# unslothai/unsloth

Hardware: AMD Instinct MI355X
Metric: train tokens/sec, Llama-3-8B QLoRA (NF4) r=16 seq2048 bf16 (higher is better)
Workload: dtype bf16; 1 GPU; Llama-3-8B QLoRA NF4 r=16 (q,k,v,o,gate,up,down) seq2048 bf16, fwd+bwd+AdamW; model=Llama-3-8B (synthetic weights), global_batch=4, seq_len=2048, parallelism=dp1, layers=32, lora_rank=16, gradient_checkpointing=unsloth, gc_schedule_chosen=all (every layer keeps everything), nf4_decoded_weight_mirrors=off (every NF4 weight is decoded at every use INSIDE the timed step), trainable_params=41943040, attention=csrc/attention.hip (causal GQA flash, fwd+bwd), optimizer=FlatAdamW fp32 on LoRA params

## Files before the change

unsloth_amd/csrc/lora_side.hip:

```cpp
#include "common.h"

typedef __attribute__((ext_vector_type(2))) __bf16 bf16x2_t;
typedef __attribute__((ext_vector_type(2))) _Float16 f16x2_t;

#define UAMD_TN_MAX_PROBLEMS 8

namespace {

constexpr int TN_COLS = 128;
constexpr int TN_R = 16;

struct TnArgs {
    int n_probs;
    int M;
    int S;
    int rows_per_wave;
    int total_slabs;
    int slab_start[UAMD_TN_MAX_PROBLEMS + 1];
    int64_t ws_off[UAMD_TN_MAX_PROBLEMS];
    float* ws;
    uamd_lora_tn_problem p[UAMD_TN_MAX_PROBLEMS];
};

typedef __attribute__((ext_vector_type(8))) __bf16 bf16x8_t;
// ... 31 lines not shown
#endif
constexpr int TN_NST = UAMD_TN_STAGES;
static_assert(TN_NST >= 2 && TN_NST <= 4, "ring of 2..4 stages (4 x 4 x 10 KiB = the 160 KiB of a CU)");
constexpr int TN_WAVE_LDS = TN_NST * TN_STAGE;

__device__ __forceinline__ void tn_dma(const void* gptr, unsigned lds_dst) {
    unsigned keep;
    asm volatile(
        "s_mov_b32 %0, m0\n\t"
        "s_mov_b32 m0, %2\n\t"
        "s_nop 0\n\t"
        "global_load_lds_dwordx4 %1, off\n\t"
        "s_mov_b32 m0, %0"
        : "=&s"(keep)
        : "v"(gptr), "s"(lds_dst)
        : "memory");
}

template <typename T>
__global__ void __launch_bounds__(256) lora_tn_kernel(TnArgs a) {
    extern __shared__ __attribute__((aligned(16))) unsigned char smem[];
    typedef typename Mfma16<T>::frag frag_t;
    const int tid = threadIdx.x, lane = tid & 63;
    const int wave = __builtin_amdgcn_readfirstlane(tid >> 6);
    const int64_t unit = (int64_t)blockIdx.x * 4 + wave;
    if (unit >= (int64_t)a.total_slabs * a.S) return;
    const int slab_lin = (int)(unit % a.total_slabs);
    const int sblk = (int)(unit / a.total_slabs);
    int pi = 0;
#pragma unroll
    for (int i = 1; i < UAMD_TN_MAX_PROBLEMS; ++i)
        if (i < a.n_probs && slab_lin >= a.slab_start[i]) pi = i;
    const uamd_lora_tn_problem& pr = a.p[pi];
    const int slab = slab_lin - a.slab_start[pi];
    const int n_slabs = a.slab_start[pi + 1] - a.slab_start[pi];
    const int M = a.M, N = pr.N, R = pr.R;
    const T* Z = (const T*)pr.Z;
    const float* P = pr.P;
    unsigned char* my = smem + wave * TN_WAVE_LDS;
    const unsigned my_lds = (unsigned)(uintptr_t)(lds_u8*)my;

    const int zr4 = lane >> 4;
    int zcol[8];
#pragma unroll
    for (int i = 0; i < 8; ++i) {
        const int row = 4 * i + zr4;
        const int f = (row & 3) | (((row >> 3) & 1) << 2);
        const int u16 = ((((lane & 15) >> 1) ^ f) << 1) | (lane & 1);
        int col = slab * TN_COLS + u16 * 8;
        if (col + 8 > N) col = N - 8;
        zcol[i] = col;
    }
    const int prow = lane >> 2;
    const int pc = (lane & 3) * 4 + 4 <= ((R + 3) & ~3) ? (lane & 3) * 4 : 0;
    auto issue = [&](int m0, int stage) {
        const unsigned d = my_lds + stage * TN_STAGE;
#pragma unroll
        for (int i = 0; i < 8; ++i) {
            int row = m0 + 4 * i + zr4;
            row = row < M ? row : M - 1;
            tn_dma(Z + (int64_t)row * pr.ldz + zcol[i], d + i * 1024);
        }
#pragma unroll
        for (int i = 0; i < 2; ++i) {
            int row = m0 + 16 * i + prow;
            row = row < M ? row : M - 1;
            tn_dma(P + (int64_t)row * pr.ldp + pc, d + TN_ZT + i * 1024);
        }
    };

    const int l15 = lane & 15, g4 = lane >> 4;
    const int sg2 = l15 >> 2;
    const int f_rd = sg2 | ((g4 & 1) << 2);
    const int z_lane = (8 * g4 + sg2) * 256 + f_rd * 32 + (l15 & 3) * 8;
    const int p_lane = TN_ZT + (8 * g4) * 64 + l15 * 4;

    f32x4_t acc[8];
#pragma unroll
    for (int j = 0; j < 8; ++j) acc[j] = f32x4_t{0.f, 0.f, 0.f, 0.f};

    const int m_base = sblk * a.rows_per_wave;
    const int m_end = min(m_base + a.rows_per_wave, M);
    const int nch = (m_end - m_base + 31) / 32;
#pragma unroll
    for (int i = 0; i < TN_NST - 1; ++i)
        if (i < nch) issue(m_base + 32 * i, i);
    for (int ch = 0; ch < nch; ++ch) {
        const int m0 = m_base + ch * 32;
        const int stage = ch % TN_NST;
        if (ch + TN_NST - 1 < nch) {
            issue(m0 + 32 * (TN_NST - 1), (ch + TN_NST - 1) % TN_NST);
            if (TN_NST == 2) asm volatile("s_waitcnt vmcnt(10)" ::: "memory");
            else if (TN_NST == 3) asm volatile("s_waitcnt vmcnt(20)" ::: "memory");
            else asm volatile("s_waitcnt vmcnt(30)" ::: "memory");
        } else {
            const int younger = nch - 1 - ch;
            if (younger >= 2) asm volatile("s_waitcnt vmcnt(20)" ::: "memory");
            else if (younger == 1) asm volatile("s_waitcnt vmcnt(10)" ::: "memory");
            else asm volatile("s_waitcnt vmcnt(0)" ::: "memory");
        }
        const unsigned char* sz = my + stage * TN_STAGE;
        union { T e[8]; frag_t f; } pa;
#pragma unroll
        for (int e = 0; e < 8; ++e) {
            float x = *reinterpret_cast<const float*>(sz + p_lane + e * 64);
            if (m0 + 8 * g4 + e >= M || l15 >= R) x = 0.f;
            pa.e[e] = from_f32<T>(x);
        }
#pragma unroll
        for (int jt = 0; jt < 8; ++jt) {
            union { s16x4_t h[2]; frag_t f; } zb;
            const int a0 = z_lane ^ (jt * 32);
            zb.h[0] = __builtin_amdgcn_ds_read_tr16_b64_v4i16((lds_s16x4*)(sz + a0));
            zb.h[1] = __builtin_amdgcn_ds_read_tr16_b64_v4i16((lds_s16x4*)(sz + a0 + 4 * 256));
            acc[jt] = Mfma16<T>::run(pa.f, zb.f, acc[jt]);
        }
    }

    const int64_t npad = (int64_t)n_slabs * TN_COLS;
    float* part = a.ws + a.ws_off[pi] + (int64_t)sblk * TN_R * npad + slab * TN_COLS + l15;
#pragma unroll
    for (int jt = 0; jt < 8; ++jt)
#pragma unroll
        for (int r = 0; r < 4; ++r) part[(int64_t)(4 * g4 + r) * npad + jt * 16] = acc[jt][r];
}

__global__ void __launch_bounds__(256) lora_tn_reduce_kernel(TnArgs a) {
    const int pi = blockIdx.y;
    const uamd_lora_tn_problem& pr = a.p[pi];
    const int n_slabs = a.slab_start[pi + 1] - a.slab_start[pi];
    const int64_t npad = (int64_t)n_slabs * TN_COLS;
    const int64_t idx = (int64_t)blockIdx.x * 256 + threadIdx.x;
    const int N = pr.N, R = pr.R;
    if (idx >= (int64_t)R * N) return;
    const int r = (int)(idx / N), n = (int)(idx - (int64_t)r * N);
    const float* part = a.ws + a.ws_off[pi] + (int64_t)r * npad + n;
    float v = 0.f;
    const int64_t sstride = (int64_t)TN_R * npad;
    int s = 0;
    for (; s + 8 <= a.S; s += 8) {
        float t[8];
#pragma unroll
        for (int u = 0; u < 8; ++u) t[u] = part[(int64_t)(s + u) * sstride];
#pragma unroll
        for (int u = 0; u < 8; ++u) v += t[u];
    }
    for (; s < a.S; ++s) v += part[(int64_t)s * sstride];
    v *= pr.scale;
    float* o = (pr.out_nr & 1) ? pr.out + (int64_t)n * pr.ldo + r : pr.out + (int64_t)r * pr.ldo + n;
    *o = (pr.out_nr & 2) ? *o + v : v;
}

constexpr int XA_KS = 64;
constexpr int XA_XT = 32 * XA_KS * 2;
template <int NT> struct XaCfg {
    static constexpr int WT = NT * 16 * XA_KS * 2;
    static constexpr int STAGE = XA_XT + WT;
    static constexpr int WAVE = 2 * STAGE;
    static constexpr int RED = 4 * 32 * NT * 16 * 4;
    static constexpr int LDS = 4 * WAVE > RED ? 4 * WAVE : RED;
};

template <typename T, int NT>
__global__ void __launch_bounds__(256) lora_xa2_kernel(const T* __restrict__ X, int64_t ldx,
                                                       const T* __restrict__ W, int64_t ldw,
                                                       float* __restrict__ out, int64_t ld_out,
                                                       T* __restrict__ out_k, int64_t ld_k, int k_cols,
                                                       int M, int K, int R, int out_cols) {
    extern __shared__ __attribute__((aligned(16))) unsigned char smem[];
    typedef typename Mfma16<T>::frag frag_t;
    typedef XaCfg<NT> C;
    const int tid = threadIdx.x, lane = tid & 63;
    const int wave = __builtin_amdgcn_readfirstlane(tid >> 6);
    const int l15 = lane & 15, g4 = lane >> 4;
    const int m0 = blockIdx.x * 32;
    unsigned char* my = smem + wave * C::WAVE;
    const unsigned my_lds = (unsigned)(uintptr_t)(lds_u8*)my;

    const int nsteps_all = (K + XA_KS - 1) / XA_KS;
    const int s_beg = (nsteps_all * wave) / 4, s_end = (nsteps_all * (wave + 1)) / 4;

    const int drow = lane >> 3;
    int xoff[4], woff[2 * NT];
    int xslot[4];
#pragma unroll
    for (int i = 0; i < 4; ++i) {
        const int row = 8 * i + drow;
        xslot[i] = (lane & 7) ^ ((row >> 1) & 7);
        int gm = m0 + row;
        gm = gm < M ? gm : M - 1;
        xoff[i] = gm;
    }
    int wslot[2 * NT];
#pragma unroll
    for (int i = 0; i < 2 * NT; ++i) {
        const int row = 8 * i + drow;
        wslot[i] = (lane & 7) ^ ((row >> 1) & 7);
        woff[i] = row < R ? row : R - 1;
    }
    auto issue = [&](int step, int stage) {
        const unsigned d = my_lds + stage * C::STAGE;
        const int k0 = step * XA_KS;
#pragma unroll
        for (int i = 0; i < 4; ++i) {
            int k = k0 + xslot[i] * 8;
            k = k + 8 <= K ? k : K - 8;
            tn_dma(X + (int64_t)xoff[i] * ldx + k, d + i * 1024);
        }
#pragma unroll
        for (int i = 0; i < 2 * NT; ++i) {
            int k = k0 + wslot[i] * 8;
            k = k + 8 <= K ? k : K - 8;
            tn_dma(W + (int64_t)woff[i] * ldw + k, d + XA_XT + i * 1024);
        }
    };

    f32x4_t acc[2][NT];
#pragma unroll
    for (int i = 0; i < 2; ++i)
#pragma unroll
        for (int j = 0; j < NT; ++j) acc[i][j] = f32x4_t{0.f, 0.f, 0.f, 0.f};

    const int sw = (l15 >> 1) & 7;
    const int f_lane = l15 * 128;
    constexpr int NDMA = 4 + 2 * NT;
    const int nst = s_end - s_beg;
    const int rot = nst > 0 ? (int)(blockIdx.x % nst) : 0;
    auto step_of = [&](int i) { const int j = i + rot; return s_beg + (j >= nst ? j - nst : j); };
    if (nst > 0) issue(step_of(0), 0);
    for (int it = 0; it < nst; ++it) {
        const int st = step_of(it);
        const int stage = it & 1;
        if (it + 1 < nst) {
            issue(step_of(it + 1), stage ^ 1);
            if (NDMA == 6) asm volatile("s_waitcnt vmcnt(6)" ::: "memory");
            else if (NDMA == 8) asm volatile("s_waitcnt vmcnt(8)" ::: "memory");
            else if (NDMA == 10) asm volatile("s_waitcnt vmcnt(10)" ::: "memory");
            else asm volatile("s_waitcnt vmcnt(12)" ::: "memory");
        } else {
            asm volatile("s_waitcnt vmcnt(0)" ::: "memory");
        }
        const unsigned char* sx = my + stage * C::STAGE;
        const unsigned char* swt = sx + XA_XT;
        const bool tail = st * XA_KS + XA_KS > K;
#pragma unroll
        for (int ks = 0; ks < 2; ++ks) {
            const int slot = ((4 * ks + g4) ^ sw) * 16;
            union FU { uint4 r; frag_t f; };
            FU xa[2], wb[NT];
#pragma unroll
            for (int i = 0; i < 2; ++i) xa[i].r = *reinterpret_cast<const uint4*>(sx + i * 2048 + f_lane + slot);
#pragma unroll
            for (int j = 0; j < NT; ++j) wb[j].r = *reinterpret_cast<const uint4*>(swt + j * 2048 + f_lane + slot);
            if (tail) {
                if (st * XA_KS + ks * 32 + g4 * 8 + 8 > K) {
#pragma unroll
                    for (int i = 0; i < 2; ++i) xa[i].r = make_uint4(0, 0, 0, 0);
                }
            }
#pragma unroll
            for (int i = 0; i < 2; ++i)
#pragma unroll
                for (int j = 0; j < NT; ++j) acc[i][j] = Mfma16<T>::run(xa[i].f, wb[j].f, acc[i][j]);
        }
    }

    __syncthreads();
    float* red = reinterpret_cast<float*>(smem);
#pragma unroll
    for (int i = 0; i < 2; ++i)
#pragma unroll
        for (int j = 0; j < NT; ++j)
#pragma unroll
            for (int r = 0; r < 4; ++r)
                red[(wave * 32 + i * 16 + 4 * g4 + r) * (NT * 16) + j * 16 + l15] = acc[i][j][r];
    __syncthreads();
    if (out != nullptr) {
        for (int idx = tid; idx < 32 * out_cols; idx += 256) {
            const int mm = idx / out_cols, c = idx - mm * out_cols;
            if (m0 + mm < M) {
                float v = 0.f;
                if (c < R) {
                    const float* q = red + mm * (NT * 16) + c;
                    v = ((q[0] + q[32 * NT * 16]) + q[2 * 32 * NT * 16]) + q[3 * 32 * NT * 16];
                }
                out[(int64_t)(m0 + mm) * ld_out + c] = v;
            }
        }
    }
    if (out_k != nullptr) {
        const int vec_per_row = k_cols >> 3;
        for (int idx = tid; idx < 32 * vec_per_row; idx += 256) {
            const int mm = idx / vec_per_row, c0 = (idx - mm * vec_per_row) * 8;
            if (m0 + mm < M) {
                Vec16<T> v;
#pragma unroll
                for (int j = 0; j < 8; ++j) {
                    const int c = c0 + j;
                    float x = 0.f;
                    if (c < R) {
                        const float* q = red + mm * (NT * 16) + c;
                        x = ((q[0] + q[32 * NT * 16]) + q[2 * 32 * NT * 16]) + q[3 * 32 * NT * 16];
                    }
                    v.e[j] = from_f32<T>(x);
                }
                st16(out_k + (int64_t)(m0 + mm) * ld_k + c0, v);
            }
        }
    }
}

template <typename T, int NT>
int launch_xa2(const void* X, int64_t ldx, const void* W, int64_t ldw, float* out, int64_t ld_out, void* out_k,
               int64_t ld_k, int k_cols, int M, int K, int R, int out_cols, hipStream_t st) {
    return uamd_launch_lds<&lora_xa2_kernel<T, NT>>(dim3((unsigned)((M + 31) / 32)), dim3(256), XaCfg<NT>::LDS, st, (const T*)X, ldx,
                                                    (const T*)W, ldw, out, ld_out, (T*)out_k, ld_k, k_cols, M, K, R, out_cols);
}

template <typename T>
int xa2_dispatch(const void* X, int64_t ldx, const void* W, int64_t ldw, float* out, int64_t ld_out, void* out_k,
                 int64_t ld_k, int k_cols, int M, int K, int R, int out_cols, hipStream_t st) {
    const int nt = (R + 15) / 16;
    if (nt <= 1) return launch_xa2<T, 1>(X, ldx, W, ldw, out, ld_out, out_k, ld_k, k_cols, M, K, R, out_cols, st);
    if (nt <= 2) return launch_xa2<T, 2>(X, ldx, W, ldw, out, ld_out, out_k, ld_k, k_cols, M, K, R, out_cols, st);
    if (nt <= 3) return launch_xa2<T, 3>(X, ldx, W, ldw, out, ld_out, out_k, ld_k, k_cols, M, K, R, out_cols, st);
    if (nt <= 4) return launch_xa2<T, 4>(X, ldx, W, ldw, out, ld_out, out_k, ld_k, k_cols, M, K, R, out_cols, st);
    return UAMD_ERR_ARG;
}

}

extern "C" int uamd_lora_tn(const uamd_lora_tn_problem* probs, int n_probs, int M, float* workspace,
                            int64_t workspace_floats, int dtype, void* stream) {
    if (!probs || n_probs < 1 || n_probs > UAMD_TN_MAX_PROBLEMS || M < 0 || !workspace) return UAMD_ERR_ARG;
    if (M == 0) return UAMD_OK;
    TnArgs a;
    a.n_probs = n_probs; a.M = M; a.ws = workspace;
    {
        int64_t slabs_all = 0;
        for (int i = 0; i < n_probs; ++i) slabs_all += (probs[i].N + TN_COLS - 1) / TN_COLS;
        int rpw = UAMD_TN_RPW_MAX;
        while (rpw > 128 && slabs_all * ((M + rpw - 1) / rpw) < UAMD_TN_MIN_WAVES) rpw >>= 1;
        a.rows_per_wave = rpw;
        a.S = (M + rpw - 1) / rpw;
    }
    int slabs = 0;
    int64_t off = 0;
    int max_rn_blocks = 1;
    for (int i = 0; i < UAMD_TN_MAX_PROBLEMS; ++i) {
        a.slab_start[i] = slabs;
        if (i < n_probs) {
            const uamd_lora_tn_problem& p = probs[i];
            if (!p.P || !p.Z || !p.out || p.N <= 0 || p.R <= 0 || p.R > TN_R) return UAMD_ERR_ARG;
            if ((p.N & 7) || p.N < 8 || (p.ldz & 7) || (p.ldp & 3) || !aligned16(p.Z) || !aligned16(p.P)) return UAMD_ERR_ALIGN;
            a.p[i] = p;
            a.ws_off[i] = off;
            const int ns = (p.N + TN_COLS - 1) / TN_COLS;
            slabs += ns;
            off += (int64_t)a.S * TN_R * ns * TN_COLS;
            const int64_t rn = ((int64_t)p.R * p.N + 255) / 256;
            if (rn > max_rn_blocks) max_rn_blocks = (int)rn;
        } else {
            a.p[i] = probs[0];
            a.ws_off[i] = 0;
        }
    }
    a.slab_start[UAMD_TN_MAX_PROBLEMS] = slabs;
    for (int i = n_probs; i < UAMD_TN_MAX_PROBLEMS; ++i) a.slab_start[i + 1] = slabs;
    a.total_slabs = slabs;
    if (off > workspace_floats) return UAMD_ERR_ARG;
    const int64_t blocks = ((int64_t)slabs * a.S + 3) / 4;
    if (blocks > 0x7fffffffLL) return UAMD_ERR_ARG;
    hipStream_t st = (hipStream_t)stream;
    UAMD_DISPATCH_HALF(dtype,
        if (int rc = uamd_launch_lds<&lora_tn_kernel<T>>(dim3((unsigned)blocks), dim3(256), 4 * TN_WAVE_LDS, st, a)) return rc)
    hipLaunchKernelGGL(lora_tn_reduce_kernel, dim3((unsigned)max_rn_blocks, (unsigned)n_probs), dim3(256), 0, st, a);
    return uamd_launch_status();
}

extern "C" int uamd_lora_xa2k(const void* X, int64_t ldx, const void* W, int64_t ldw, float* out, int64_t ld_out,
                              void* out_k, int64_t ld_k, int k_cols, int M, int K, int R, int out_cols, int dtype,
                              void* stream) {
    if (M < 0 || K < 8 || R <= 0 || R > 64) return UAMD_ERR_ARG;
    if (!out && !out_k) return UAMD_ERR_ARG;
    if (out && (out_cols < R || out_cols > 256)) return UAMD_ERR_ARG;
    if (out_k && (k_cols < R || k_cols > 256)) return UAMD_ERR_ARG;
    if (M == 0) return UAMD_OK;
    if ((K & 7) || (ldx & 7) || (ldw & 7) || !aligned16(X) || !aligned16(W)) return UAMD_ERR_ALIGN;
    if (out_k && ((k_cols & 7) || (ld_k & 7) || !aligned16(out_k))) return UAMD_ERR_ALIGN;
    UAMD_DISPATCH_HALF(dtype, return xa2_dispatch<T>(X, ldx, W, ldw, out, ld_out, out_k, ld_k, k_cols, M, K, R, out_cols, (hipStream_t)stream))
    return UAMD_ERR_DTYPE;
}

extern "C" int uamd_lora_xa2(const void* X, int64_t ldx, const void* W, int64_t ldw, float* out, int64_t ld_out,
                             int M, int K, int R, int out_cols, int dtype, void* stream) {
    if (!out) return UAMD_ERR_ARG;
    return uamd_lora_xa2k(X, ldx, W, ldw, out, ld_out, nullptr, 0, 0, M, K, R, out_cols, dtype, stream);
}

namespace {
template <typename T>
__global__ void __launch_bounds__(256) lora_prepare_kernel(const uamd_lora_prep_desc* __restrict__ d, int n_mats,
                                                          const int* __restrict__ tile_prefix) {
    __shared__ float tile[32][33];
    int lo = 0, hi = n_mats - 1;
    const int bid = blockIdx.x;
    while (lo < hi) {
        const int mid = (lo + hi + 1) >> 1;
        if (tile_prefix[mid] <= bid) lo = mid; else hi = mid - 1;
    }
    const uamd_lora_prep_desc m = d[lo];
    const int t = bid - tile_prefix[lo];
    const int tiles_c = (m.cols + 31) / 32;
    const int r0 = (t / tiles_c) * 32, c0 = (t % tiles_c) * 32;
    const int tx = threadIdx.x & 31, ty = threadIdx.x >> 5;
    const float* src = (const float*)m.src;
    T* rm = (T*)m.dst_rowmajor;
    T* tr = (T*)m.dst_transposed;
    T* pad = (T*)m.dst_pad;
    const bool pad_t = m.pad_transposed != 0;
#pragma unroll
    for (int i = 0; i < 4; ++i) {
        const int r = r0 + ty + 8 * i, c = c0 + tx;
        float v = 0.f;
        if (r < m.rows && c < m.cols) {
            v = src[(int64_t)r * m.cols + c];
            if (rm) rm[(int64_t)r * m.cols + c] = from_f32<T>(v);
            if (pad && !pad_t) pad[(int64_t)r * m.pad_ld + c] = from_f32<T>(m.pad_scale * v);
        }
        tile[ty + 8 * i][tx] = v;
    }
    __syncthreads();
    if (tr || (pad && pad_t)) {
#pragma unroll
        for (int i = 0; i < 4; ++i) {
            const int c = c0 + ty + 8 * i, r = r0 + tx;
            if (r < m.rows && c < m.cols) {
                const float v = tile[tx][ty + 8 * i];
                if (tr) tr[(int64_t)c * m.rows + r] = from_f32<T>(v);
                if (pad && pad_t) pad[(int64_t)c * m.pad_ld + r] = from_f32<T>(m.pad_scale * v);
            }
        }
    }
}
}

extern "C" int uamd_lora_prepare(const uamd_lora_prep_desc* descs_dev, const int* tile_prefix_dev, int n_mats,
                                 int total_tiles, int dtype, void* stream) {
    if (!descs_dev || !tile_prefix_dev || n_mats <= 0 || total_tiles < 0) return UAMD_ERR_ARG;
    if (total_tiles == 0) return UAMD_OK;
    hipStream_t st = (hipStream_t)stream;
    UAMD_DISPATCH_HALF(dtype, hipLaunchKernelGGL((lora_prepare_kernel<T>), dim3((unsigned)total_tiles), dim3(256), 0, st, descs_dev, n_mats,
                                                 tile_prefix_dev))
    return uamd_launch_status();
}
```

unsloth_amd/kernels/utils.py:

```python
import ctypes
import os

import torch

from .. import _lib
from .. import nf4 as _nf4
from .._lib import GemmGroup

MAX_FUSED_SIZE = 65536
next_power_of_2 = lambda n: 1 << (max(int(n), 1) - 1).bit_length()

FUSED_NF4 = True
FUSED_NF4_MAX_M = 512
GEMM256_MODE = "auto"
GEMM256_MIN_TILES = 160
LORA_XA_V2 = True
LORA_XA_MAX_RANKS = 192


def calculate_settings(n):
    BLOCK_SIZE = next_power_of_2(n)
    num_warps = 4
    if BLOCK_SIZE >= 32768:
        num_warps = 32
# ... 60 lines not shown


def get_lora_parameters_bias(proj):
    base_layer = getattr(proj, "base_layer", proj)
    W = base_layer.weight
    W_quant = _resolve_quant_state(base_layer, W)
    if getattr(proj, "disable_adapters", True) or proj.merged:
        return W, W_quant, None, None, None, base_layer.bias
    adapter = getattr(proj, "active_adapters", None)
    if adapter is None:
        adapter = getattr(proj, "active_adapter", ("default"))
    adapter = adapter[0]
    return (W, W_quant, proj.lora_A[adapter].weight, proj.lora_B[adapter].weight,
            proj.scaling[adapter], base_layer.bias)


@torch.inference_mode()
def fast_dequantize(W, quant_state=None, out=None, use_global_buffer=False):
    if quant_state is None:
        return W
    _refuse_fp8([(W,)])
    is_transposed = W.shape[0] == 1
    packed = W.t() if is_transposed else W
    out = _nf4.dequantize_nf4(packed, quant_state, out=out, use_global_buffer=use_global_buffer)
    return out.t() if is_transposed else out


def _group(B, C, N, ldb, absmax=None, xa=None, ld_xa=0, lb=None, R=0, scale=0.0, xk=None, bk=None, bias=None):
    return GemmGroup(
        B=B.data_ptr(), C=C.data_ptr(), absmax=absmax.data_ptr() if absmax is not None else None,
        lora_xa=xa.data_ptr() if xa is not None else None, lora_b=lb.data_ptr() if lb is not None else None,
        ldb=ldb, ldc=C.stride(0), ld_xa=ld_xa, ld_lb=lb.stride(0) if lb is not None else 0,
        N=N, R=R, lora_scale=float(scale), _pad=0,
        lora_xk=xk.data_ptr() if xk is not None else None, lora_bk=bk.data_ptr() if bk is not None else None,
        ld_xk=xk.stride(0) if xk is not None else 0, ld_bk=bk.stride(0) if bk is not None else 0,
        Rk=xk.shape[1] if xk is not None else 0, _pad2=0, bias=bias.data_ptr() if bias is not None else None)


def _use_gemm256(M, K, Ns):
    if GEMM256_MODE == "off" or K % 64:
        return False
    if GEMM256_MODE == "on":
        return True
    cols = sum((n + 255) // 256 for n in Ns)
    return ((M + 255) // 256) * cols >= GEMM256_MIN_TILES or ((M + 127) // 128) * cols >= GEMM256_MIN_TILES


GEMM_SPAN_LIMIT = 1 << 32


def _chunk_rows(row_bytes, align):
    rows = (GEMM_SPAN_LIMIT - 1) // max(row_bytes, 1) // align * align
    if rows < align:
        raise RuntimeError(f"unsloth_amd: a GEMM operand row of {row_bytes} bytes leaves no whole {align}-row chunk "
                           f"below the {GEMM_SPAN_LIMIT}-byte span limit")
    return rows


def _row_spans(M, row_bytes, align):
    if M * row_bytes < GEMM_SPAN_LIMIT:
        return [(0, M)]
    step = _chunk_rows(row_bytes, align)
    return [(r0, min(step, M - r0)) for r0 in range(0, M, step)]


def _launch_gemm(X2d, groups, nf4, accumulate=False, nn=False):
    M, K = X2d.shape
    prologue_lora = any(g.lora_xa and not g.lora_xk for g in groups)
    if nn:
        name = "uamd_gemm_nn_256"
    elif nf4:
        name = "uamd_gemm_nt_nf4"
    elif _use_gemm256(M, K, [g.N for g in groups]) and not prologue_lora:
        name = "uamd_gemm_nt_256"
    else:
        name = "uamd_gemm_nt"
    item = X2d.element_size()
    row_bytes = X2d.stride(0) * item
    for g in groups:
        if g.lora_xk:
            row_bytes = max(row_bytes, g.ld_xk * item)
        if g.lora_xa:
            row_bytes = max(row_bytes, g.ld_xa * 4)
    for r0, rows in _row_spans(M, row_bytes, 256):
        chunk = []
        for g in groups:
            c = GemmGroup.from_buffer_copy(g)
            if r0:
                c.C += r0 * c.ldc * item
                if c.lora_xk:
                    c.lora_xk += r0 * c.ld_xk * item
                if c.lora_xa:
                    c.lora_xa += r0 * c.ld_xa * 4
            chunk.append(c)
        arr = (GemmGroup * len(chunk))(*chunk)
        _lib.call(name, X2d, ctypes.c_void_p(X2d.data_ptr() + r0 * X2d.stride(0) * item), X2d.stride(0), rows, K, arr,
                  len(chunk), int(accumulate), _lib.dtype_code(X2d.dtype), _lib.stream_of(X2d))
    return name


def _aligned_rows(W):
    return W.stride(1) == 1 and W.stride(0) % 8 == 0 and W.data_ptr() % 16 == 0


def _aligned_copy(W, dtype=None):
    Wc = W.to(dtype if dtype is not None else W.dtype).contiguous()
    return Wc.clone() if Wc.data_ptr() % 16 else Wc


def _rows2d(X):
    X2d = X.reshape(-1, X.shape[-1])
    return X2d if _aligned_rows(X2d) else _aligned_copy(X2d)


def _out2d(C, M, N, dtype, name):
    if not isinstance(C, torch.Tensor) or not C.is_cuda or C.dtype != dtype:
        raise ValueError(f"{name}: expected a {dtype} tensor on the GPU, got {getattr(C, 'dtype', type(C))}")
    C2 = C
    if C.dim() != 2 and C.dim() >= 1 and C.shape[-1] == N and C.numel() == M * N:
        try:
            C2 = C.view(M, N)
        except RuntimeError:
            raise ValueError(f"{name}: shape {tuple(C.shape)} with strides {C.stride()} is no [{M}, {N}] row-major matrix") \
                from None
    if C2.dim() != 2 or tuple(C2.shape) != (M, N):
        raise ValueError(f"{name}: shape {tuple(C.shape)}, expected [{M}, {N}]")
    if N > 1 and C2.stride(1) != 1:
        raise ValueError(f"{name}: column stride {C2.stride(1)}, the GEMM writes rows of unit column stride")
    return C2


import weakref
_CAST_CACHE = {}
_CAST_EPOCH = [0]


def invalidate_cast_cache(*_a, **_k):
    _CAST_EPOCH[0] += 1


try:
    from torch.optim.optimizer import register_optimizer_step_post_hook as _reg_hook
    _reg_hook(invalidate_cast_cache)
except Exception:
    pass


class _PreparedFactors:

    def __init__(self, device, dtype):
        self.device, self.dtype = device, dtype
        self.params = {}
        self.pad_bufs = {}
        self.epoch = -1
        self.table = None

    @staticmethod
    def _tiles(P):
        return ((P.shape[0] + 31) // 32) * ((P.shape[1] + 31) // 32)

    _DESC = [("src", "<u8"), ("rm", "<u8"), ("tr", "<u8"), ("rows", "<i4"), ("cols", "<i4"), ("pad", "<u8"),
             ("pad_ld", "<i8"), ("pad_scale", "<f4"), ("pad_t", "<i4")]

    def _launch(self, ents):
        import numpy as np
        key = tuple((P.data_ptr(), P.shape[0], P.shape[1], rm.data_ptr(), tr.data_ptr(),
                     None if pad is None else (pad[0].data_ptr(), pad[0].stride(0)) + tuple(pad[1:]))
                    for (P, rm, tr, pad) in ents) if len(ents) > 1 else None
        tab = self.table
        if key is None or tab is None or tab[4] != key:
            descs = np.zeros(len(ents), dtype=np.dtype(self._DESC))
            assert descs.dtype.itemsize == 56
            prefix, tot = np.zeros(len(ents), dtype=np.int32), 0
            for i, (P, rm, tr, pad) in enumerate(ents):
                if pad is None:
                    descs[i] = (P.data_ptr(), rm.data_ptr(), tr.data_ptr(), P.shape[0], P.shape[1], 0, 0, 0.0, 0)
                else:
                    buf, col, scale, transposed = pad
                    descs[i] = (P.data_ptr(), rm.data_ptr(), tr.data_ptr(), P.shape[0], P.shape[1],
                                buf.data_ptr() + col * buf.element_size(), buf.stride(0), scale, int(transposed))
                prefix[i] = tot
                tot += self._tiles(P)
            sig = descs.tobytes()
            if tab is None or tab[0] != sig:
                d = torch.from_numpy(descs.view(np.uint8).copy()).to(self.device)
                pf = torch.from_numpy(prefix).to(self.device)
                tab = (sig, d, pf, tot, key)
            else:
                tab = tab[:4] + (key,)
            if len(ents) > 1:
                self.table = tab
        any_p = ents[0][0]
        _lib.call("uamd_lora_prepare", any_p, _lib.ptr(tab[1]), _lib.ptr(tab[2]), len(ents), tab[3],
                  _lib.dtype_code(self.dtype), _lib.stream_of(any_p))

    def _forget(self, pid):
        self.params.pop(pid, None)
        for k in [k for k in self.pad_bufs if pid in k[0]]:
            self.pad_bufs.pop(k, None)

    def _entry(self, P, padspec=None):
        pid = id(P)
        ent = self.params.get(pid)
        epoch = _CAST_EPOCH[0]
        with torch.no_grad():
            if ent is None or ent[0]() is not P or ent[1].shape != P.shape:
                rm = torch.empty(P.shape, dtype=self.dtype, device=self.device)
                tr = torch.empty((P.shape[1], P.shape[0]), dtype=self.dtype, device=self.device)
                ent = [weakref.ref(P, lambda _, pid=pid: self._forget(pid)), rm, tr, -1, -1, None]
                self.params[pid] = ent
            if padspec is not None:
                old = ent[5]
                if old is None or old[0] is not padspec[0] or old[1:] != padspec[1:]:
                    ent[5] = padspec
                    ent[4] = -1
            if self.epoch != epoch:
                live = []
                for e in list(self.params.values()):
                    Q = e[0]()
                    if Q is not None:
                        live.append((Q, e[1], e[2], e[5]))
                        e[3], e[4] = Q._version, epoch
                self._launch(live)
                self.epoch = epoch
            elif ent[4] != epoch or ent[3] != P._version:
                self._launch([(P, ent[1], ent[2], ent[5])])
                ent[3], ent[4] = P._version, epoch
        return ent

    def get(self, P, tag):
        ent = self._entry(P)
        return ent[1] if tag == "rowmajor" else ent[2]

    def get_pad(self, members, rows, width, transposed, by_rows=False):
        key = (tuple(id(P) for P, _, _ in members), rows, width, bool(transposed), bool(by_rows))
        buf = self.pad_bufs.get(key)
        if buf is None:
            buf = self.pad_bufs[key] = torch.zeros((rows, width), dtype=self.dtype, device=self.device)
        for P, off, scale in members:
            self._entry(P, (buf, int(off) * (width if by_rows else 1), float(scale), bool(transposed)))
        return buf


_PREPARED = {}


def _preparable(P, dtype):
    return (isinstance(P, torch.nn.Parameter) and P.is_cuda and P.dtype == torch.float32 and P.dim() == 2
            and P.is_contiguous() and dtype in (torch.bfloat16, torch.float16))


def _prepared_for(device, dtype):
    g = _PREPARED.get((device, dtype))
    if g is None:
        g = _PREPARED[(device, dtype)] = _PreparedFactors(device, dtype)
    return g


def _cached_cast(P, tag, dtype, build):
    if not isinstance(P, torch.nn.Parameter):
        return build()
    if tag in ("rowmajor", "T") and _preparable(P, dtype):
        return _prepared_for(P.device, dtype).get(P, tag)
    pid = id(P)
    ent = _CAST_CACHE.get(pid)
    if (ent is None or ent[0]() is not P or ent[1] != P._version or ent[2] != P.data_ptr()
            or ent[3] != _CAST_EPOCH[0]):
        ent = (weakref.ref(P, lambda _, pid=pid: _CAST_CACHE.pop(pid, None)), P._version, P.data_ptr(),
               _CAST_EPOCH[0], {})
        _CAST_CACHE[pid] = ent
    key = (tag, dtype)
    out = ent[4].get(key)
    if out is None:
        with torch.no_grad():
            out = build()
        ent[4][key] = out
    return out


def rank_block_bk(members, rows, width, transposed, dtype, by_rows=False):
    if not all(_preparable(P, dtype) for P, _, _ in members):
        with torch.no_grad():
            buf = torch.zeros((rows, width), dtype=dtype, device=members[0][0].device)
            for P, off, scale in members:
                src = P.detach().t() if transposed else P.detach()
                val = (src.float() * float(scale)).to(dtype)
                if by_rows:
                    buf[off:off + src.shape[0], :src.shape[1]] = val
                else:
                    buf[:, off:off + src.shape[1]] = val
        return buf
    return _prepared_for(members[0][0].device, dtype).get_pad(members, rows, width, transposed, by_rows)


def lora_xa(X2d, A_list, out=None, out_k=None, k_cols=0):
    dtype = X2d.dtype
    Rs = [A.shape[0] for A in A_list]
    Rp = [(r + 7) // 8 * 8 for r in Rs]
    K = X2d.shape[1]
    if len(A_list) == 1 and Rs[0] == Rp[0]:
        Acat = cast_lora(A_list[0], dtype)
    else:
        def _cat():
            if Rs == Rp:
                return torch.cat([cast_lora(A, dtype) for A in A_list], dim=0)
            buf = torch.zeros((sum(Rp), K), dtype=dtype, device=X2d.device)
            o = 0
            for A, r, rp in zip(A_list, Rs, Rp):
                buf[o:o + r] = A
                o += rp
            return buf
        if all(isinstance(A, torch.nn.Parameter) for A in A_list):
            tag = ("cat",) + tuple((id(A), A._version, A.data_ptr()) for A in A_list[1:])
            Acat = _cached_cast(A_list[0], tag, dtype, _cat)
        else:
            Acat = _cat()
    Rt = Acat.shape[0]
    if out is None:
        out = torch.empty((X2d.shape[0], Rt), dtype=torch.float32, device=X2d.device)
    else:
        assert out.dtype == torch.float32 and tuple(out.shape) == (X2d.shape[0], Rt) and out.stride(1) == 1 \
            and out.stride(0) % 4 == 0
    if Rt > LORA_XA_MAX_RANKS:
        assert out_k is None, "the rank-block output takes <= 64 ranks per launch (_xa_and_rank_block groups them)"
        if not _aligned_rows(Acat):
            Acat = _aligned_copy(Acat)
        for c0 in range(0, Rt, LORA_XA_MAX_RANKS):
            rc = min(LORA_XA_MAX_RANKS, Rt - c0)
            lora_xa(X2d, [Acat[c0:c0 + rc]], out=out[:, c0:c0 + rc])
    elif out_k is not None:
        assert Rt <= 64 and out_k.dtype == dtype and out_k.stride(1) == 1 and k_cols >= Rt
        _lib.call("uamd_lora_xa2k", X2d, _lib.ptr(X2d), X2d.stride(0), _lib.ptr(Acat), Acat.stride(0), _lib.ptr(out),
                  out.stride(0), _lib.ptr(out_k), out_k.stride(0), k_cols, X2d.shape[0], K, Rt, Rt,
                  _lib.dtype_code(dtype), _lib.stream_of(X2d))
    else:
        _lib.call("uamd_lora_xa2" if (LORA_XA_V2 and Rt <= 64 and K >= 8) else "uamd_lora_xa", X2d,
                  _lib.ptr(X2d), X2d.stride(0), _lib.ptr(Acat), Acat.stride(0), _lib.ptr(out), out.stride(0),
                  X2d.shape[0], K, Rt, Rt, _lib.dtype_code(dtype), _lib.stream_of(X2d))
    offs, o = [], 0
    for rp in Rp:
        offs.append((o, rp))
        o += rp
    return out, offs


def cast_lora(P, dtype):
    return _cached_cast(P, "rowmajor", dtype, lambda: P.to(dtype).contiguous())


def cast_lora_t(P, dtype):
    return _cached_cast(P, "T", dtype, lambda: P.to(dtype).t().contiguous())


def _pad_rank(B, Rp, dtype):
    N, r = B.shape
    if r == Rp:
        return cast_lora(B, dtype)
    out = torch.zeros((N, Rp), dtype=dtype, device=B.device)
    out[:, :r] = B
    return out


def _rank_width(r):
    return (r + 63) // 64 * 64


def _xa_and_rank_block(X2d, A_list, want_k, out=None):
    Rt = sum((A.shape[0] + 7) // 8 * 8 for A in A_list)
    if not want_k:
        xa, offs = lora_xa(X2d, A_list, out=out)
        return xa, offs, None
    M = X2d.shape[0]
    width = _rank_width(Rt)
    if Rt <= 64 and LORA_XA_V2 and X2d.shape[1] >= 8:
        xk = torch.empty((M, width), dtype=X2d.dtype, device=X2d.device)
        xa, offs = lora_xa(X2d, A_list, out=out, out_k=xk, k_cols=width)
    elif (LORA_XA_V2 and X2d.shape[1] >= 8 and Rt <= 192
          and all(A.shape[0] % 8 == 0 and A.shape[0] <= 64 for A in A_list)):
        xk = torch.empty((M, width), dtype=X2d.dtype, device=X2d.device)
        xa = out if out is not None else torch.empty((M, Rt), dtype=torch.float32, device=X2d.device)
        groups, cur, cur_r = [], [], 0
        for A in A_list:
            if cur and cur_r + A.shape[0] > 64:
                groups.append((cur, cur_r))
                cur, cur_r = [], 0
            cur.append(A)
            cur_r += A.shape[0]
        groups.append((cur, cur_r))
        offs, col = [], 0
        for gi, (As, r) in enumerate(groups):
            last = gi == len(groups) - 1
            _, o = lora_xa(X2d, As, out=xa[:, col:col + r], out_k=xk[:, col:], k_cols=(width - col) if last else r)
            offs += [(col + a, b) for a, b in o]
            col += r
    else:
        xa, offs = lora_xa(X2d, A_list, out=out)
        xk = torch.zeros((M, width), dtype=X2d.dtype, device=X2d.device)
        xk[:, :Rt] = xa
    return xa, offs, xk


def _fused_nf4(q, M, K):
    return q is not None and FUSED_NF4 and M < FUSED_NF4_MAX_M and q.blocksize == 64 and K % 64 == 0


def _decoded_as(Wd, dtype):
    if Wd.dtype != dtype:
        raise TypeError(f"quant_state.dtype {Wd.dtype} != activation dtype {dtype}: the dequantised weight would be "
                        "misread by the GEMM (set quant_state.dtype to the compute dtype)")
    return Wd


def lora_linear_forward(X, projs, outs=None, return_xa=False, pre_xa=None):
    _refuse_fp8(projs)
    _lib.require_gpu(X)
    dtype = X.dtype
    if dtype not in (torch.bfloat16, torch.float16):
        raise NotImplementedError("the MFMA GEMM path takes bf16/fp16 activations")
    X2d = _rows2d(X)
    M, K = X2d.shape
    lead = X.shape[:-1]
    biases = [(p[5] if len(p) > 5 else None) for p in projs]
    projs = [tuple(p[:5]) for p in projs]
    with_lora = [p for p in projs if p[2] is not None]
    Ns = [(q.shape[0] if q is not None else W.shape[0]) for (W, q, _, _, _) in projs]
    fused_nf4 = [_fused_nf4(q, M, K) for (_, q, _, _, _) in projs]
    dense_Ns = [n for n, f in zip(Ns, fused_nf4) if not f]
    use256 = bool(dense_Ns) and _use_gemm256(M, K, dense_Ns)
    xa, offs, xk = None, [], None
    if with_lora and pre_xa is not None:
        xa, offs, xk = pre_xa
        if (xk is not None) != use256:
            xa, offs, xk = _xa_and_rank_block(X2d, [p[2] for p in with_lora], use256)
    elif with_lora:
        xa, offs, xk = _xa_and_rank_block(X2d, [p[2] for p in with_lora], use256)
    results, dense_groups, nf4_groups, keep = [], [], [], []
    resident = None
    if len(projs) > 1 and all(q is not None and _nf4.mirror_wanted(q) for (_, q, _, _, _) in projs) and not any(fused_nf4):
        _, resident = _nf4.resident_group([p_[0] for p_ in projs], [p_[1] for p_ in projs])
    decoded = {}
    if resident is None:
        todo = [gi for gi, (W, q, _, _, _) in enumerate(projs) if q is not None and not fused_nf4[gi]]
        if len(todo) > 1 and all(projs[gi][1].dtype == dtype and projs[gi][1].quant_type == "nf4" for gi in todo):
            slots = [_nf4.scratch(X.device, projs[gi][1].shape[0] * projs[gi][1].shape[1], dtype, slot=8 + gi).view(
                tuple(projs[gi][1].shape)) for gi in todo]
            _nf4.dequantize_nf4_group([projs[gi][0] for gi in todo], [projs[gi][1] for gi in todo], slots)
            decoded = dict(zip(todo, slots))
    li = 0
    for gi, (W, W_quant, A, B, s) in enumerate(projs):
        if W_quant is not None:
            assert W_quant.shape[1] == K, "weight/in_features mismatch"
        N = Ns[gi]
        C = _out2d(outs[gi], M, N, dtype, f"outs[{gi}]") if outs is not None else torch.empty((M, N), dtype=dtype, device=X.device)
        kw = {}
        if biases[gi] is not None:
            bias = biases[gi].detach()
            if bias.dtype != dtype or not bias.is_contiguous():
                bias = bias.to(dtype).contiguous()
            assert bias.numel() == N
            keep.append(bias)
            kw["bias"] = bias
        if A is not None:
            o, rp = offs[li]
            li += 1
            if xk is not None and not fused_nf4[gi]:
# ... 510 lines not shown
```

Baseline: 38220 tokens/s.

## Generalize LoRA XA kernel to multi-stage ring and stack prepared A weights

Templatizes the X·Aᵀ LoRA kernel on row tiles and pipeline depth. Rank-16 problems (NT=1) now use 16-row tiles with a 3-stage DMA ring, which doubles the block count and deepens the prefetch. Separately, concatenated A matrices are served from one persistent stacked bf16 buffer that the prepared-cast cache writes into directly, instead of a cached torch.cat copy. The risks are smaller tiles loading the same A weights more often, and more LDS per block.

```diff
diff --git a/unsloth_amd/csrc/lora_side.hip b/unsloth_amd/csrc/lora_side.hip
--- a/unsloth_amd/csrc/lora_side.hip
+++ b/unsloth_amd/csrc/lora_side.hip
@@ -207,28 +207,38 @@
 }
 
 constexpr int XA_KS = 64;
-constexpr int XA_XT = 32 * XA_KS * 2;
-template <int NT> struct XaCfg {
+template <int NT, int RT, int NS> struct XaCfg {
+    static constexpr int ROWS = 16 * RT;
+    static constexpr int XT = ROWS * XA_KS * 2;
     static constexpr int WT = NT * 16 * XA_KS * 2;
-    static constexpr int STAGE = XA_XT + WT;
-    static constexpr int WAVE = 2 * STAGE;
-    static constexpr int RED = 4 * 32 * NT * 16 * 4;
+    static constexpr int STAGE = XT + WT;
+    static constexpr int WAVE = NS * STAGE;
+    static constexpr int RED = 4 * ROWS * NT * 16 * 4;
     static constexpr int LDS = 4 * WAVE > RED ? 4 * WAVE : RED;
+    static constexpr int NDMA = 2 * RT + 2 * NT;
+    static_assert(NS >= 2 && NDMA * (NS - 1) <= 63, "the counted wait has 6 bits");
+    static_assert(LDS <= 160 * 1024, "the ring must fit the LDS of a CU");
 };
 
-template <typename T, int NT>
-__global__ void __launch_bounds__(256) lora_xa2_kernel(const T* __restrict__ X, int64_t ldx,
-                                                       const T* __restrict__ W, int64_t ldw,
-                                                       float* __restrict__ out, int64_t ld_out,
-                                                       T* __restrict__ out_k, int64_t ld_k, int k_cols,
-                                                       int M, int K, int R, int out_cols) {
-    extern __shared__ __attribute__((aligned(16))) unsigned char smem[];
+template <int N> __device__ __forceinline__ void xa_wait() { asm volatile("s_waitcnt vmcnt(%0)" ::"n"(N) : "memory"); }
+
+struct XaArgs {
+    const void* X; const void* W; float* out; void* out_k;
+    int64_t ldx, ldw, ld_out, ld_k;
+    int K, R, out_cols, k_cols;
+};
+template <typename T, int NT, int RT, int NS>
+__device__ __forceinline__ void xa2_tile(const XaArgs& a, int M, int tile, unsigned char* smem) {
     typedef typename Mfma16<T>::frag frag_t;
-    typedef XaCfg<NT> C;
+    typedef XaCfg<NT, RT, NS> C;
+    const T* __restrict__ X = (const T*)a.X;
+    const T* __restrict__ W = (const T*)a.W;
+    const int64_t ldx = a.ldx, ldw = a.ldw;
+    const int K = a.K, R = a.R;
     const int tid = threadIdx.x, lane = tid & 63;
     const int wave = __builtin_amdgcn_readfirstlane(tid >> 6);
     const int l15 = lane & 15, g4 = lane >> 4;
-    const int m0 = blockIdx.x * 32;
+    const int m0 = tile * C::ROWS;
     unsigned char* my = smem + wave * C::WAVE;
     const unsigned my_lds = (unsigned)(uintptr_t)(lds_u8*)my;
 
@@ -236,10 +246,10 @@
     const int s_beg = (nsteps_all * wave) / 4, s_end = (nsteps_all * (wave + 1)) / 4;
 
     const int drow = lane >> 3;
-    int xoff[4], woff[2 * NT];
-    int xslot[4];
-#pragma unroll
-    for (int i = 0; i < 4; ++i) {
+    int xoff[2 * RT], woff[2 * NT];
+    int xslot[2 * RT];
+#pragma unroll
+    for (int i = 0; i < 2 * RT; ++i) {
         const int row = 8 * i + drow;
         xslot[i] = (lane & 7) ^ ((row >> 1) & 7);
         int gm = m0 + row;
@@ -257,7 +267,7 @@
         const unsigned d = my_lds + stage * C::STAGE;
         const int k0 = step * XA_KS;
 #pragma unroll
-        for (int i = 0; i < 4; ++i) {
+        for (int i = 0; i < 2 * RT; ++i) {
             int k = k0 + xslot[i] * 8;
             k = k + 8 <= K ? k : K - 8;
             tn_dma(X + (int64_t)xoff[i] * ldx + k, d + i * 1024);
@@ -266,78 +276,92 @@
         for (int i = 0; i < 2 * NT; ++i) {
             int k = k0 + wslot[i] * 8;
             k = k + 8 <= K ? k : K - 8;
-            tn_dma(W + (int64_t)woff[i] * ldw + k, d + XA_XT + i * 1024);
+            tn_dma(W + (int64_t)woff[i] * ldw + k, d + C::XT + i * 1024);
         }
     };
 
-    f32x4_t acc[2][NT];
-#pragma unroll
-    for (int i = 0; i < 2; ++i)
+    f32x4_t acc[RT][NT];
+#pragma unroll
+    for (int i = 0; i < RT; ++i)
 #pragma unroll
         for (int j = 0; j < NT; ++j) acc[i][j] = f32x4_t{0.f, 0.f, 0.f, 0.f};
 
     const int sw = (l15 >> 1) & 7;
     const int f_lane = l15 * 128;
-    constexpr int NDMA = 4 + 2 * NT;
-    const int nst = s_end - s_beg;
-    const int rot = nst > 0 ? (int)(blockIdx.x % nst) : 0;
-    auto step_of = [&](int i) { const int j = i + rot; return s_beg + (j >= nst ? j - nst : j); };
-    if (nst > 0) issue(step_of(0), 0);
-    for (int it = 0; it < nst; ++it) {
-        const int st = step_of(it);
-        const int stage = it & 1;
-        if (it + 1 < nst) {
-            issue(step_of(it + 1), stage ^ 1);
-            if (NDMA == 6) asm volatile("s_waitcnt vmcnt(6)" ::: "memory");
-            else if (NDMA == 8) asm volatile("s_waitcnt vmcnt(8)" ::: "memory");
-            else if (NDMA == 10) asm volatile("s_waitcnt vmcnt(10)" ::: "memory");
-            else asm volatile("s_waitcnt vmcnt(12)" ::: "memory");
-        } else {
-            asm volatile("s_waitcnt vmcnt(0)" ::: "memory");
-        }
+    auto multiply = [&](int st, int stage) {
         const unsigned char* sx = my + stage * C::STAGE;
-        const unsigned char* swt = sx + XA_XT;
+        const unsigned char* swt = sx + C::XT;
         const bool tail = st * XA_KS + XA_KS > K;
 #pragma unroll
         for (int ks = 0; ks < 2; ++ks) {
             const int slot = ((4 * ks + g4) ^ sw) * 16;
             union FU { uint4 r; frag_t f; };
-            FU xa[2], wb[NT];
-#pragma unroll
-            for (int i = 0; i < 2; ++i) xa[i].r = *reinterpret_cast<const uint4*>(sx + i * 2048 + f_lane + slot);
+            FU xa[RT], wb[NT];
+#pragma unroll
+            for (int i = 0; i < RT; ++i) xa[i].r = *reinterpret_cast<const uint4*>(sx + i * 2048 + f_lane + slot);
 #pragma unroll
             for (int j = 0; j < NT; ++j) wb[j].r = *reinterpret_cast<const uint4*>(swt + j * 2048 + f_lane + slot);
             if (tail) {
                 if (st * XA_KS + ks * 32 + g4 * 8 + 8 > K) {
 #pragma unroll
-                    for (int i = 0; i < 2; ++i) xa[i].r = make_uint4(0, 0, 0, 0);
+                    for (int i = 0; i < RT; ++i) xa[i].r = make_uint4(0, 0, 0, 0);
                 }
             }
 #pragma unroll
-            for (int i = 0; i < 2; ++i)
+            for (int i = 0; i < RT; ++i)
 #pragma unroll
                 for (int j = 0; j < NT; ++j) acc[i][j] = Mfma16<T>::run(xa[i].f, wb[j].f, acc[i][j]);
         }
-    }
-
+    };
+    const int nst = s_end - s_beg;
+    const int rot = nst > 0 ? (int)((m0 >> 5) % nst) : 0;
+    auto step_of = [&](int i) { const int j = i + rot; return s_beg + (j >= nst ? j - nst : j); };
+#pragma unroll
+    for (int p = 0; p < NS - 1; ++p)
+        if (p < nst) issue(step_of(p), p);
+    int it = 0, stage = 0;
+    for (; it + NS - 1 < nst; ++it) {
+        issue(step_of(it + NS - 1), stage == 0 ? NS - 1 : stage - 1);
+        xa_wait<C::NDMA * (NS - 1)>();
+        multiply(step_of(it), stage);
+        stage = stage + 1 == NS ? 0 : stage + 1;
+    }
+    auto drain = [&](auto left) {
+        constexpr int U = decltype(left)::value;
+        if (nst > U) {
+            xa_wait<C::NDMA * U>();
+            multiply(step_of(nst - 1 - U), stage);
+            stage = stage + 1 == NS ? 0 : stage + 1;
+        }
+    };
+    if constexpr (NS >= 4) drain(std::integral_constant<int, 2>{});
+    if constexpr (NS >= 3) drain(std::integral_constant<int, 1>{});
+    drain(std::integral_constant<int, 0>{});
+    static_assert(NS <= 4, "the count-down above is written out for rings of 2..4 stages");
+
+    float* __restrict__ out = a.out;
+    T* __restrict__ out_k = (T*)a.out_k;
+    const int64_t ld_out = a.ld_out, ld_k = a.ld_k;
+    const int out_cols = a.out_cols, k_cols = a.k_cols;
+    constexpr int QS = C::ROWS * NT * 16;
     __syncthreads();
     float* red = reinterpret_cast<float*>(smem);
 #pragma unroll
-    for (int i = 0; i < 2; ++i)
+    for (int i = 0; i < RT; ++i)
 #pragma unroll
         for (int j = 0; j < NT; ++j)
 #pragma unroll
             for (int r = 0; r < 4; ++r)
-                red[(wave * 32 + i * 16 + 4 * g4 + r) * (NT * 16) + j * 16 + l15] = acc[i][j][r];
+                red[(wave * C::ROWS + i * 16 + 4 * g4 + r) * (NT * 16) + j * 16 + l15] = acc[i][j][r];
     __syncthreads();
     if (out != nullptr) {
-        for (int idx = tid; idx < 32 * out_cols; idx += 256) {
+        for (int idx = tid; idx < C::ROWS * out_cols; idx += 256) {
             const int mm = idx / out_cols, c = idx - mm * out_cols;
             if (m0 + mm < M) {
                 float v = 0.f;
                 if (c < R) {
                     const float* q = red + mm * (NT * 16) + c;
-                    v = ((q[0] + q[32 * NT * 16]) + q[2 * 32 * NT * 16]) + q[3 * 32 * NT * 16];
+                    v = ((q[0] + q[QS]) + q[2 * QS]) + q[3 * QS];
                 }
                 out[(int64_t)(m0 + mm) * ld_out + c] = v;
             }
@@ -345,7 +369,7 @@
     }
     if (out_k != nullptr) {
         const int vec_per_row = k_cols >> 3;
-        for (int idx = tid; idx < 32 * vec_per_row; idx += 256) {
+        for (int idx = tid; idx < C::ROWS * vec_per_row; idx += 256) {
             const int mm = idx / vec_per_row, c0 = (idx - mm * vec_per_row) * 8;
             if (m0 + mm < M) {
                 Vec16<T> v;
@@ -355,7 +379,7 @@
                     float x = 0.f;
                     if (c < R) {
                         const float* q = red + mm * (NT * 16) + c;
-                        x = ((q[0] + q[32 * NT * 16]) + q[2 * 32 * NT * 16]) + q[3 * 32 * NT * 16];
+                        x = ((q[0] + q[QS]) + q[2 * QS]) + q[3 * QS];
                     }
                     v.e[j] = from_f32<T>(x);
                 }
@@ -365,22 +389,23 @@
     }
 }
 
+template <typename T, int NT, int RT, int NS>
+__global__ void __launch_bounds__(256) lora_xa2_kernel(XaArgs a, int M) {
+    extern __shared__ __attribute__((aligned(16))) unsigned char smem[];
+    xa2_tile<T, NT, RT, NS>(a, M, (int)blockIdx.x, smem);
+}
+
+template <int NT> struct XaPlan {
+    static constexpr int RT = NT == 1 ? 1 : 2;
+    static constexpr int NS = NT == 1 ? 3 : 2;
+};
+
 template <typename T, int NT>
-int launch_xa2(const void* X, int64_t ldx, const void* W, int64_t ldw, float* out, int64_t ld_out, void* out_k,
-               int64_t ld_k, int k_cols, int M, int K, int R, int out_cols, hipStream_t st) {
-    return uamd_launch_lds<&lora_xa2_kernel<T, NT>>(dim3((unsigned)((M + 31) / 32)), dim3(256), XaCfg<NT>::LDS, st, (const T*)X, ldx,
-                                                    (const T*)W, ldw, out, ld_out, (T*)out_k, ld_k, k_cols, M, K, R, out_cols);
-}
-
-template <typename T>
-int xa2_dispatch(const void* X, int64_t ldx, const void* W, int64_t ldw, float* out, int64_t ld_out, void* out_k,
-                 int64_t ld_k, int k_cols, int M, int K, int R, int out_cols, hipStream_t st) {
-    const int nt = (R + 15) / 16;
-    if (nt <= 1) return launch_xa2<T, 1>(X, ldx, W, ldw, out, ld_out, out_k, ld_k, k_cols, M, K, R, out_cols, st);
-    if (nt <= 2) return launch_xa2<T, 2>(X, ldx, W, ldw, out, ld_out, out_k, ld_k, k_cols, M, K, R, out_cols, st);
-    if (nt <= 3) return launch_xa2<T, 3>(X, ldx, W, ldw, out, ld_out, out_k, ld_k, k_cols, M, K, R, out_cols, st);
-    if (nt <= 4) return launch_xa2<T, 4>(X, ldx, W, ldw, out, ld_out, out_k, ld_k, k_cols, M, K, R, out_cols, st);
-    return UAMD_ERR_ARG;
+int launch_xa2(const XaArgs& a, int M, hipStream_t st) {
+    typedef XaPlan<NT> P;
+    typedef XaCfg<NT, P::RT, P::NS> C;
+    return uamd_launch_lds<&lora_xa2_kernel<T, NT, P::RT, P::NS>>(dim3((unsigned)((M + C::ROWS - 1) / C::ROWS)), dim3(256), C::LDS,
+                                                                  st, a, M);
 }
 
 }
@@ -443,7 +468,14 @@
     if (M == 0) return UAMD_OK;
     if ((K & 7) || (ldx & 7) || (ldw & 7) || !aligned16(X) || !aligned16(W)) return UAMD_ERR_ALIGN;
     if (out_k && ((k_cols & 7) || (ld_k & 7) || !aligned16(out_k))) return UAMD_ERR_ALIGN;
-    UAMD_DISPATCH_HALF(dtype, return xa2_dispatch<T>(X, ldx, W, ldw, out, ld_out, out_k, ld_k, k_cols, M, K, R, out_cols, (hipStream_t)stream))
+    const XaArgs a{X, W, out, out_k, ldx, ldw, ld_out, ld_k, K, R, out_cols, k_cols};
+    hipStream_t st = (hipStream_t)stream;
+    const int nt = (R + 15) / 16;
+    UAMD_DISPATCH_HALF(dtype,
+        if (nt <= 1) return launch_xa2<T, 1>(a, M, st);
+        if (nt <= 2) return launch_xa2<T, 2>(a, M, st);
+        if (nt <= 3) return launch_xa2<T, 3>(a, M, st);
+        return launch_xa2<T, 4>(a, M, st))
     return UAMD_ERR_DTYPE;
 }
 
diff --git a/unsloth_amd/kernels/utils.py b/unsloth_amd/kernels/utils.py
--- a/unsloth_amd/kernels/utils.py
+++ b/unsloth_amd/kernels/utils.py
@@ -236,6 +236,7 @@
         self.device, self.dtype = device, dtype
         self.params = {}
         self.pad_bufs = {}
+        self.stacks = {}
         self.epoch = -1
         self.table = None
 
@@ -282,6 +283,8 @@
         self.params.pop(pid, None)
         for k in [k for k in self.pad_bufs if pid in k[0]]:
             self.pad_bufs.pop(k, None)
+        for k in [k for k in self.stacks if pid in k]:
+            self.stacks.pop(k, None)
 
     def _entry(self, P, padspec=None):
         pid = id(P)
@@ -316,6 +319,33 @@
         ent = self._entry(P)
         return ent[1] if tag == "rowmajor" else ent[2]
 
+    @staticmethod
+    def stack_plan(shapes):
+        if not shapes or any(len(s) != 2 or s[1] != shapes[0][1] or s[0] <= 0 for s in shapes):
+            return None
+        offs, o = [], 0
+        for r, _ in shapes:
+            offs.append(o)
+            o += r
+        return offs, (o, shapes[0][1])
+
+    def get_stack(self, members):
+        ents = [self._entry(P) for P in members]
+        offs, shape = self.stack_plan([tuple(P.shape) for P in members])
+        key = tuple(id(P) for P in members)
+        st = self.stacks.get(key)
+        row_bytes = shape[1] * torch.empty((), dtype=self.dtype).element_size()
+        if (st is not None and tuple(st.shape) == shape
+                and all(e[1].data_ptr() == st.data_ptr() + o * row_bytes for e, o in zip(ents, offs))):
+            return st
+        st = self.stacks[key] = torch.empty(shape, dtype=self.dtype, device=self.device)
+        for P, e, o in zip(members, ents, offs):
+            e[1] = st[o:o + P.shape[0]]
+            e[4] = -1
+        for P in members:
+            self._entry(P)
+        return st
+
     def get_pad(self, members, rows, width, transposed, by_rows=False):
         key = (tuple(id(P) for P, _, _ in members), rows, width, bool(transposed), bool(by_rows))
         buf = self.pad_bufs.get(key)
@@ -394,7 +424,9 @@
                 buf[o:o + r] = A
                 o += rp
             return buf
-        if all(isinstance(A, torch.nn.Parameter) for A in A_list):
+        if Rs == Rp and all(_preparable(A, dtype) and A.shape[1] == K for A in A_list):
+            Acat = _prepared_for(A_list[0].device, dtype).get_stack(A_list)
+        elif all(isinstance(A, torch.nn.Parameter) for A in A_list):
             tag = ("cat",) + tuple((id(A), A._version, A.data_ptr()) for A in A_list[1:])
             Acat = _cached_cast(A_list[0], tag, dtype, _cat)
         else:
```

Result: no change. 38310 tokens/s, median of 6 (+0.2%).
